# marcin119a/vae-los-angeles

Hardware: AMD Instinct MI355X
Metric: training samples/sec, MultiModalVAE batch 65536 (higher is better)
Workload: dtype bf16

## Files before the change

vae-los-angeles_amd/csrc/gemm_nt2.h:

```cpp
#pragma once
#include "common.h"
#include "gemm_nt_epi.h"

namespace mm {

template <int WN> struct Nt2Lds {
    static constexpr int A_BYTES = TILE * ROW_BYTES;
    static constexpr int W_BYTES = 64 * WN * ROW_BYTES;
    static constexpr int SLOT = A_BYTES + W_BYTES;
    static constexpr int RING = 2 * SLOT;
    static constexpr int RED = RING;
    static constexpr int ECOL = RED + 4 * 64 * WN * 4;
    static constexpr int TOTAL = ECOL + 8 * 64 * WN * 4;
};

STAMP_BUFFER(nt2)

typedef __attribute__((address_space(3))) void lds_void;
typedef __attribute__((address_space(1))) const void gbl_void;

template <typename Epi, int WN>
__device__ __forceinline__ void nt2_loss_epilogue(unsigned char* smem, const float* ecol, float* red, f32x4 (&acc)[4][4], const Epi& epi,
                                                  int row0, int col0, int M, int N, int tid, int lane, int wr, int wc)
{
    static_assert(WN == 2, "128 x 128 tiles: the fp32 tile is exactly the 64 KB ring");
    const int li = lane & 15, lg = lane >> 4;
    const int c = tid & 31, r0 = tid >> 5;
    const int colg = col0 + 4 * c;
    typedef typename Epi::t_t TT;
    const TT* __restrict__ T = epi.T;
    bf16* __restrict__ G = epi.G;
    const bool interior = row0 + TILE <= M && col0 + 128 <= N;
    float t[16][4];
    if (interior) {
#pragma unroll
        for (int i = 0; i < 16; ++i) {
            const TT* tp = T + (long)(row0 + r0 + 8 * i) * epi.ldt + colg;
#pragma unroll
            for (int e = 0; e < 4; e += Epi::VT) VLoad<TT, Epi::VT>::ld(tp + e, &t[i][e]);
        }
    } else {
#pragma unroll
        for (int i = 0; i < 16; ++i) {
            const TT* tp = T + (long)min(row0 + r0 + 8 * i, M - 1) * epi.ldt;
#pragma unroll
            for (int e = 0; e < 4; e += Epi::VT) VLoad<TT, Epi::VT>::ld(tp + min(colg + e, N - Epi::VT), &t[i][e]);
        }
    }
    __syncthreads();
#pragma unroll
    for (int m = 0; m < 4; ++m)
#pragma unroll
        for (int n = 0; n < 4; ++n) {
            const int row = wr * 64 + m * 16 + li, ch = 16 * wc + 4 * n + lg;
            *(f32x4*)(smem + row * 512 + ((ch ^ (row & 7)) << 4)) = acc[m][n];
        }
    __syncthreads();
    const int gcols = (int)min((long)((N + 7) & ~7), epi.ldg);
    const unsigned char* src = smem + r0 * 512 + ((c ^ (r0 & 7)) << 4);
    const f32x2 b01 = {ecol[4 * c], ecol[4 * c + 1]}, b23 = {ecol[4 * c + 2], ecol[4 * c + 3]};
    f32x2 lsum2 = {0.f, 0.f};
    if (interior) {
#pragma unroll
        for (int i = 0; i < 16; ++i) {
            const f32x4 z = *(const f32x4*)(src + i * 8 * 512);
            f32x2 g01, g23;
            lsum2 += epi.term2(f32x2{z[0], z[1]} + b01, f32x2{t[i][0], t[i][1]}, g01);
            lsum2 += epi.term2(f32x2{z[2], z[3]} + b23, f32x2{t[i][2], t[i][3]}, g23);
            const bf16x4 o = {(bf16)g01[0], (bf16)g01[1], (bf16)g23[0], (bf16)g23[1]};
            *(bf16x4*)(G + (long)(row0 + r0 + 8 * i) * epi.ldg + colg) = o;
        }
    } else {
#pragma unroll
        for (int i = 0; i < 16; ++i) {
            const int grow = row0 + r0 + 8 * i;
            const f32x4 z = *(const f32x4*)(src + i * 8 * 512);
            f32x2 g01, g23;
            const f32x2 l01 = epi.term2(f32x2{z[0], z[1]} + b01, f32x2{t[i][0], t[i][1]}, g01);
            const f32x2 l23 = epi.term2(f32x2{z[2], z[3]} + b23, f32x2{t[i][2], t[i][3]}, g23);
            const float l[4] = {l01[0], l01[1], l23[0], l23[1]}, ge[4] = {g01[0], g01[1], g23[0], g23[1]};
            float g[4];
#pragma unroll
            for (int e = 0; e < 4; ++e) {
                const bool ok = grow < M && colg + e < N;
                lsum2[e & 1] += ok ? l[e] : 0.f;
                g[e] = ok ? ge[e] : 0.f;
            }
            if (grow < M && colg < gcols) {
                bf16x4 o;
#pragma unroll
                for (int e = 0; e < 4; ++e) o[e] = (bf16)g[e];
                *(bf16x4*)(G + (long)grow * epi.ldg + colg) = o;
            }
        }
    }
    const float lsum = lsum2[0] + lsum2[1];
    const float ws = wave_sum(lsum);
    if (lane == 0) red[tid >> 6] = ws;
    __syncthreads();
    if (tid == 0) {
        const double v = (double)red[0] + (double)red[1] + (double)red[2] + (double)red[3];
        if (v != 0.0) unsafeAtomicAdd(epi.sum, v);
    }
}

template <typename Epi, int WN>
__device__ __forceinline__ void nt2_relumask_epilogue(unsigned char* smem, f32x4 (&acc)[4][4], const Epi& epi,
                                                      int row0, int col0, int M, int N, int tid, int lane, int wr, int wc)
{
    static_assert(WN == 2, "128 x 128 tiles: the fp32 tile is exactly the 64 KB ring");
    const int li = lane & 15, lg = lane >> 4;
    const int c = tid & 31, r0 = tid >> 5;
    const int colg = col0 + 4 * c;
    const bf16* __restrict__ H = epi.H;
    bf16* __restrict__ C = epi.C;
    const int ch_ = min(colg, ((N + 7) & ~7) - 4);
    bf16x4 hv[16];
#pragma unroll
    for (int i = 0; i < 16; ++i) hv[i] = *(const bf16x4*)(H + (long)min(row0 + r0 + 8 * i, M - 1) * epi.ldh + ch_);
    __syncthreads();
#pragma unroll
    for (int m = 0; m < 4; ++m)
#pragma unroll
        for (int n = 0; n < 4; ++n) {
            const int row = wr * 64 + m * 16 + li, ch = 16 * wc + 4 * n + lg;
            *(f32x4*)(smem + row * 512 + ((ch ^ (row & 7)) << 4)) = acc[m][n];
        }
    __syncthreads();
    const int ccols = (int)min((long)((N + 7) & ~7), epi.ldc);
    const unsigned char* src = smem + r0 * 512 + ((c ^ (r0 & 7)) << 4);
#pragma unroll
    for (int i = 0; i < 16; ++i) {
        const int grow = row0 + r0 + 8 * i;
        const f32x4 z = *(const f32x4*)(src + i * 8 * 512);
        bf16x4 o;
#pragma unroll
        for (int e = 0; e < 4; ++e) o[e] = (bf16)((colg + e < N && (float)hv[i][e] > 0.f) ? z[e] : 0.f);
        if (grow < M && colg < ccols) *(bf16x4*)(C + (long)grow * epi.ldc + colg) = o;
    }
    __syncthreads();
}

template <typename Epi, int WN>
__device__ __forceinline__ void nt2_bnbwd_epilogue(unsigned char* smem, const float* ecol, float* red, f32x4 (&acc)[4][4], const Epi& epi,
                                                   int row0, int col0, int M, int N, int tid, int lane, int wr, int wc)
{
    static_assert(WN == 2, "128 x 128 tiles: the fp32 tile is exactly the 64 KB ring");
    constexpr int BN = 128;
    const int li = lane & 15, lg = lane >> 4;
    const int c = tid & 31, r0 = tid >> 5;
    const int colg = col0 + 4 * c;
    const bf16* __restrict__ Y = epi.Y;
    const uint8_t* __restrict__ K_ = epi.mask;
    bf16* __restrict__ C = epi.C;
    const bool has_mask = K_ != nullptr;
    const int cy = min(colg, ((N + 7) & ~7) - 4);
    bf16x4 yv[16]; uint32_t mv[16];
#pragma unroll
    for (int i = 0; i < 16; ++i) {
        const long grow = min(row0 + r0 + 8 * i, M - 1);
        yv[i] = *(const bf16x4*)(Y + grow * epi.ldy + cy);
        mv[i] = has_mask ? *(const uint32_t*)(K_ + grow * epi.ldm + min(colg, ((N + 3) & ~3) - 4)) : 0x01010101u;
    }
    __syncthreads();
#pragma unroll
    for (int m = 0; m < 4; ++m)
#pragma unroll
        for (int n = 0; n < 4; ++n) {
            const int row = wr * 64 + m * 16 + li, ch = 16 * wc + 4 * n + lg;
            *(f32x4*)(smem + row * 512 + ((ch ^ (row & 7)) << 4)) = acc[m][n];
        }
    __syncthreads();
    const int ccols = (int)min((long)((N + 7) & ~7), epi.ldc);
    const unsigned char* src = smem + r0 * 512 + ((c ^ (r0 & 7)) << 4);
    float sc[4], sh[4], mu[4], rs[4], s1[4] = {0.f, 0.f, 0.f, 0.f}, s2[4] = {0.f, 0.f, 0.f, 0.f};
#pragma unroll
    for (int e = 0; e < 4; ++e) { sc[e] = ecol[4 * c + e]; sh[e] = ecol[BN + 4 * c + e]; mu[e] = ecol[2 * BN + 4 * c + e]; rs[e] = ecol[3 * BN + 4 * c + e]; }
#pragma unroll
    for (int i = 0; i < 16; ++i) {
        const int grow = row0 + r0 + 8 * i;
        const f32x4 z = *(const f32x4*)(src + i * 8 * 512);
        bf16x4 o;
#pragma unroll
        for (int e = 0; e < 4; ++e) {
            const bool ok = grow < M && colg + e < N;
            const float y = (float)yv[i][e];
            const float keep = ((mv[i] >> (8 * e)) & 0xffu) ? epi.inv_keep : 0.f;
            const float d = (ok && y * sc[e] + sh[e] > 0.f) ? z[e] * (has_mask ? keep : 1.f) : 0.f;
            const float xh = (y - mu[e]) * rs[e];
            s1[e] += d; s2[e] += d * xh;
            o[e] = (bf16)d;
        }
        if (grow < M && colg < ccols) *(bf16x4*)(C + (long)grow * epi.ldc + colg) = o;
    }
    __syncthreads();
    float* part = (float*)smem;
#pragma unroll
    for (int e = 0; e < 4; ++e) { part[(r0 * 2 + 0) * BN + 4 * c + e] = s1[e]; part[(r0 * 2 + 1) * BN + 4 * c + e] = s2[e]; }
    __syncthreads();
    if (tid < 2 * BN) {
        const int which = tid >> 7, col = tid & (BN - 1);
        float v = 0.f;
#pragma unroll
        for (int g = 0; g < 8; ++g) v += part[(g * 2 + which) * BN + col];
        if (col0 + col < N) unsafeAtomicAdd((which ? epi.stat2 : epi.stat1) + col0 + col, (double)v);
    }
    __syncthreads();
}

template <typename Epi, int WN>
__global__ __launch_bounds__(128 * WN, 2)
void gemm_nt2_kernel(const bf16* __restrict__ A, long lda, const bf16* __restrict__ W, long ldw, int M, int N, int K, int gx, int gy, Epi epi)
{
    typedef bf16 CT;
    typedef Nt2Lds<WN> LD;
    constexpr int BK = 64, BN = 64 * WN, NW = 2 * WN;
    constexpr int A_PIECES = TILE / 8, W_PIECES = BN / 8;
    constexpr int A_PER = A_PIECES / NW, W_PER = W_PIECES / NW;
    typedef Mma<CT>::frag frag;
    typedef EpiCols<sizeof(typename Epi::out_t) == 2> EC;
    extern __shared__ __attribute__((aligned(16))) unsigned char smem[];
    float* red = (float*)(smem + LD::RED);
    float* ecol = (float*)(smem + LD::ECOL);

    const int tid = threadIdx.x, lane = tid & 63, wid = __builtin_amdgcn_readfirstlane(tid >> 6);
    const int wr = wid / WN, wc = wid % WN;
    const int nk = (K + BK - 1) / BK;
    const int kmax = ((K + 7) & ~7) - 8;
    const int ntiles = ((gx + 7) / 8) * 8 * gy;

    auto tile_rc = [&](int T, int& rt, int& ct) { const int slot = T >> 3; ct = slot % gy; rt = (slot / gy) * 8 + (T & 7); };
    auto next_tile = [&](int T) {
        for (T += gridDim.x; T < ntiles; T += gridDim.x) { int rt, ct; tile_rc(T, rt, ct); if (rt < gx) return T; }
        return -1;
    };
    int T = blockIdx.x;
    { int rt, ct; tile_rc(T, rt, ct); if (rt >= gx) T = next_tile(T); }
    if (T < 0) return;
    const int prow = lane >> 3, ppos = lane & 7;
    auto issue = [&](int tile, int kt, int slot) {
        int rt, ct; tile_rc(tile, rt, ct);
        const int row0 = rt * TILE, col0 = ct * BN;
        unsigned char* sA = smem + slot * LD::SLOT;
        unsigned char* sW = sA + LD::A_BYTES;
        const bf16* Ak = A + kt * BK;
        const bf16* Wk = W + kt * BK;
#pragma unroll
        for (int i = 0; i < A_PER; ++i) {
            const int p = wid + NW * i;
            const int r = p * 8 + prow;
            const int c = ppos ^ (r & 7);
            const int kc = min(c * 8, kmax - kt * BK);
            const unsigned off = (unsigned)min(row0 + r, M - 1) * (unsigned)lda + (unsigned)kc;
            __builtin_amdgcn_global_load_lds((gbl_void*)(Ak + off), (lds_void*)(sA + p * 1024), 16, 0, 0);
        }
#pragma unroll
        for (int i = 0; i < W_PER; ++i) {
            const int p = wid + NW * i, r = p * 8 + prow;
            const int c = ppos ^ (r & 7);
            const int wrw = (r & ~63) + EC::wrow(r & 63);
            const unsigned off = (unsigned)(col0 + wrw) * (unsigned)ldw + (unsigned)(c * 8);
            __builtin_amdgcn_global_load_lds((gbl_void*)(Wk + off), (lds_void*)(sW + p * 1024), 16, 0, 0);
        }
    };

    f32x4 acc[4][4];
    frag f0a[4], f0b[4], f1a[4], f1b[4];
    auto rd = [&](frag (&af)[4], frag (&bf)[4], int slot, int s) {
        const unsigned char* sA = smem + slot * LD::SLOT;
        const unsigned char* sW = sA + LD::A_BYTES;
        const int ch = s * 4 + (lane >> 4);
#pragma unroll
        for (int m = 0; m < 4; ++m) {
            const int r = wr * 64 + m * 16 + (lane & 15);
            af[m] = *(const frag*)(sA + r * ROW_BYTES + ((ch ^ (r & 7)) << 4));
        }
#pragma unroll
        for (int n = 0; n < 4; ++n) { const int r = wc * 64 + n * 16 + (lane & 15); bf[n] = *(const frag*)(sW + r * ROW_BYTES + ((ch ^ (r & 7)) << 4)); }
    };
    auto mma = [&](const frag (&af)[4], const frag (&bf)[4]) {
#pragma unroll
        for (int m = 0; m < 4; ++m)
#pragma unroll
            for (int n = 0; n < 4; ++n) Mma<CT>::mma(acc[m][n], bf[n], af[m]);
    };

    STAMP_ONLY(unsigned long long st_acc[10] = {}; STAMP_T(t_begin);)
    issue(T, 0, 0);
    int g = 0;
    for (;;) {
        const int Tn = next_tile(T);
        int rt, ct; tile_rc(T, rt, ct);
        const int row0 = rt * TILE, col0 = ct * BN;
#pragma unroll
        for (int m = 0; m < 4; ++m)
#pragma unroll
            for (int n = 0; n < 4; ++n) acc[m][n] = f32x4{0.f, 0.f, 0.f, 0.f};
        EpiOperands<Epi> eops;
        for (int kt = 0; kt < nk; ++kt, ++g) {
            STAMP_T(t0);
            asm volatile("s_waitcnt vmcnt(0)" ::: "memory");
            STAMP_T(t1);
            __syncthreads();
            STAMP_T(t2);
            if (kt == 0) nt_epilogue_fill_cols<Epi, WN>(ecol, epi, col0, N, tid);
            if (kt + 1 < nk) issue(T, kt + 1, (g + 1) & 1);
            else if (Tn >= 0 && !Epi::LDS_STREAM) issue(Tn, 0, (g + 1) & 1);
            STAMP_T(t3);
            rd(f0a, f0b, g & 1, 0);
            rd(f1a, f1b, g & 1, 1);
            mma(f0a, f0b);
            mma(f1a, f1b);
            STAMP_ONLY(asm volatile("s_nop 0" :: "v"(acc[0][0][0]), "v"(acc[3][3][3])));
            STAMP_T(t4);
            STAMP_ADD(0, t1 - t0); STAMP_ADD(1, t2 - t1); STAMP_ADD(2, t3 - t2); STAMP_ADD(3, t4 - t3); STAMP_ADD(4, 1);
        }
        STAMP_T(te0);
        if (nk == 1) __syncthreads();
        if constexpr (Epi::LDS_STREAM) {
            if constexpr (Epi::MODE == 2) nt2_bnbwd_epilogue<Epi, WN>(smem, ecol, red, acc, epi, row0, col0, M, N, tid, lane, wr, wc);
            else if constexpr (Epi::MODE == 3) nt2_relumask_epilogue<Epi, WN>(smem, acc, epi, row0, col0, M, N, tid, lane, wr, wc);
            else nt2_loss_epilogue<Epi, WN>(smem, ecol, red, acc, epi, row0, col0, M, N, tid, lane, wr, wc);
            if (Tn >= 0) issue(Tn, 0, g & 1);
        } else {
            nt_epilogue_prefetch<Epi, 0>(eops, epi, row0, col0, M, N, BN, lane, wr, wc);
            nt_epilogue<CT, Epi, WN>(red, ecol, acc, epi, eops, row0, col0, M, N, tid, lane, wr, wc);
        }
        STAMP_T(te1);
        STAMP_ADD(9, te1 - te0);
        if (Tn < 0) break;
        T = Tn;
    }
    STAMP_T(t_end);
    STAMP_ADD(5, 1); STAMP_ADD(6, t_end - t_begin);
    STAMP_ONLY(if (tid == 0 && (blockIdx.x & 15) == 3) stamp_flush(stamps_nt2, st_acc));
}

template <typename Epi, int WN>
static int launch_nt2(const void* A, long lda, const void* W, long ldw, int M, int N, int K, const Epi& epi, hipStream_t st) {
    const int gx = (M + TILE - 1) / TILE, gy = (N + 64 * WN - 1) / (64 * WN);
    const int ntiles = ((gx + 7) / 8) * 8 * gy;
    int grid = NUM_CU * (WN == 2 ? 2 : 1);
    if (grid > ntiles) grid = ntiles;
    return launch_lds<gemm_nt2_kernel<Epi, WN>>(dim3(grid), dim3(128 * WN), Nt2Lds<WN>::TOTAL, st,
                                                (const bf16*)A, lda, (const bf16*)W, ldw, M, N, K, gx, gy, epi);
}

}
```

vae-los-angeles_amd/csrc/gemm_nt_epi.h:

```cpp
#pragma once
#include "common.h"
#include "wave_slab.h"

namespace mm {

template <typename OT, bool STATS_>
struct EpiStore {
    static constexpr bool STATS = STATS_;
    static constexpr bool LDS_STREAM = false;
    static constexpr int NEED = 0;
    typedef OT out_t; typedef OT h_t;
    OT* C; long ldc; const float* bias; int act; int accumulate;
    const OT* H; long ldh; const uint8_t* mask; long ldm;
    double* stat1; double* stat2;
    struct Col { float b; };
    static constexpr int NCOL = 1;
    __device__ __forceinline__ bool stores() const { return true; }
    __device__ __forceinline__ bool accum() const { return accumulate != 0; }
    bool accumulate_requested() const { return accumulate != 0; }
    __device__ __forceinline__ void fill(float* e, int BN, int cl, int c, int N) const { e[cl] = (bias && c < N) ? bias[c] : 0.f; }
    __device__ __forceinline__ Col col(const float* e, int BN, int cl) const { return Col{e[cl]}; }
    __device__ __forceinline__ int act_code() const { return act; }
    template <int ACT>
    __device__ __forceinline__ float compute(float v, float, unsigned, const Col& cc, bool count, float& s1, float& s2) const {
        v += cc.b;
        const int a = ACT < 0 ? act : ACT;
        if (a == 1) v = fmaxf(v, 0.f);
        else if (a == 2) v = __builtin_amdgcn_rcpf(1.f + __expf(-v));
        const float r = to_f32(from_f32<OT>(v));
        if (STATS && count) { s1 += r; s2 += r * r; }
        return r;
    }
};

template <typename OT, bool STATS>
inline EpiStore<OT, STATS> epi_store(const mmvae_gemm_nt_args* a) {
    return {(OT*)a->c, a->ldc, a->bias, a->act, a->accumulate, nullptr, 0, nullptr, 0, STATS ? a->stat1 : nullptr, STATS ? a->stat2 : nullptr};
}

template <typename OT, typename HT>
struct EpiReluMask {
    static constexpr bool STATS = false;
    static constexpr bool LDS_STREAM = false;
    static constexpr int NEED = 1;
    typedef OT out_t; typedef HT h_t;
    OT* C; long ldc; const HT* H; long ldh; const uint8_t* mask; long ldm;
    double* stat1; double* stat2;
    struct Col {};
    static constexpr int NCOL = 0;
    __device__ __forceinline__ bool stores() const { return true; }
    __device__ __forceinline__ bool accum() const { return false; }
    bool accumulate_requested() const { return false; }
    __device__ __forceinline__ void fill(float*, int, int, int, int) const {}
    __device__ __forceinline__ Col col(const float*, int, int) const { return Col{}; }
    __device__ __forceinline__ int act_code() const { return 0; }
    template <int ACT>
    __device__ __forceinline__ float compute(float v, float h, unsigned, const Col&, bool, float&, float&) const {
        return h > 0.f ? v : 0.f;
    }
};

template <typename OT, typename YT>
struct EpiBnBwd {
    static constexpr bool STATS = true;
    static constexpr bool LDS_STREAM = false;
    static constexpr int NEED = 2;
    typedef OT out_t; typedef YT h_t;
    OT* C; long ldc; const YT* H; long ldh; const uint8_t* mask; long ldm;
    const float* scale; const float* shift; const float* mean; const float* rstd; float inv_keep;
    const float* coef; int phase;
    double* stat1; double* stat2;
    struct Col { float sc, sh, mu, rs, c0, c1, c2; };
    __device__ __forceinline__ bool stores() const { return phase != 0; }
    __device__ __forceinline__ bool accum() const { return false; }
    bool accumulate_requested() const { return false; }
    static constexpr int NCOL = 7;
    __device__ __forceinline__ void fill(float* e, int BN, int cl, int c, int N) const {
        const bool ok = c < N, p1 = ok && phase == 1;
        e[cl] = ok ? scale[c] : 0.f; e[BN + cl] = ok ? shift[c] : 0.f; e[2 * BN + cl] = ok ? mean[c] : 0.f; e[3 * BN + cl] = ok ? rstd[c] : 0.f;
        e[4 * BN + cl] = p1 ? coef[c] : 0.f; e[5 * BN + cl] = p1 ? coef[N + c] : 0.f; e[6 * BN + cl] = p1 ? coef[2 * N + c] : 0.f;
    }
    __device__ __forceinline__ Col col(const float* e, int BN, int cl) const {
        return Col{e[cl], e[BN + cl], e[2 * BN + cl], e[3 * BN + cl], e[4 * BN + cl], e[5 * BN + cl], e[6 * BN + cl]};
    }
    __device__ __forceinline__ int act_code() const { return 0; }
    template <int ACT>
    __device__ __forceinline__ float compute(float v, float y, unsigned mb, const Col& cc, bool count, float& s1, float& s2) const {
        const float keep = mask ? (mb ? inv_keep : 0.f) : 1.f;
        const float d = (y * cc.sc + cc.sh > 0.f) ? v * keep : 0.f;
        const float xh = (y - cc.mu) * cc.rs;
        if (phase != 1) { if (count) { s1 += d; s2 += d * xh; } return d; }
        return cc.c0 * (d - cc.c1 - xh * cc.c2);
    }
};

template <int MODE_, int VT_, typename TT = float>
struct EpiLoss {
    static constexpr bool STATS = false;
    static constexpr bool LDS_STREAM = true;
    static constexpr int NEED = 0;
    static constexpr int MODE = MODE_, VT = VT_;
    typedef float out_t; typedef float h_t;
    typedef TT t_t;
    bf16* G; long ldg; const TT* T; long ldt; const float* bias; double* sum;
    struct Col { float b; };
    static constexpr int NCOL = 1;
    bool accumulate_requested() const { return false; }
    __device__ __forceinline__ void fill(float* e, int BN, int cl, int c, int N) const { e[cl] = (bias && c < N) ? bias[c] : 0.f; }
    __device__ __forceinline__ float term(float x, float t, float& g) const {
        if constexpr (MODE == 0) { const float d = x - t; g = 2.f * d; return d * d; }
        else {
            const float pe = __builtin_amdgcn_rcpf(1.f + __expf(-x));
            const float lp = fmaxf(fast_ln(pe), -100.f), l1p = fmaxf(fast_ln(1.f - pe), -100.f);
            const float pq = (1.f - pe) * pe, d = pe - t;
            g = d * fminf(pq * 1e12f, 1.f);
            return -(t * lp + (1.f - t) * l1p);
        }
    }
    __device__ __forceinline__ f32x2 term2(const f32x2 x, const f32x2 t, f32x2& g) const {
        if constexpr (MODE == 0) { const f32x2 d = x - t; g = d * 2.f; return d * d; }
        else {
            const f32x2 nx = x * -1.4426950408889634f;
            const f32x2 s = f32x2{__builtin_amdgcn_exp2f(nx[0]), __builtin_amdgcn_exp2f(nx[1])} + 1.f;
            const f32x2 pe = {__builtin_amdgcn_rcpf(s[0]), __builtin_amdgcn_rcpf(s[1])};
            const f32x2 om = 1.f - pe;
            f32x2 lp = f32x2{__builtin_amdgcn_logf(pe[0]), __builtin_amdgcn_logf(pe[1])} * 0.6931471805599453f;
            f32x2 l1p = f32x2{__builtin_amdgcn_logf(om[0]), __builtin_amdgcn_logf(om[1])} * 0.6931471805599453f;
            lp = f32x2{fmaxf(lp[0], -100.f), fmaxf(lp[1], -100.f)};
            l1p = f32x2{fmaxf(l1p[0], -100.f), fmaxf(l1p[1], -100.f)};
            const f32x2 pq = om * pe, d = pe - t, c = pq * 1e12f;
            g = d * f32x2{fminf(c[0], 1.f), fminf(c[1], 1.f)};
            return -__builtin_elementwise_fma(1.f - t, l1p, t * lp);
        }
    }
};

struct EpiBnBwdStream {
    static constexpr bool STATS = true;
    static constexpr bool LDS_STREAM = true;
    static constexpr int NEED = 0;
    static constexpr int MODE = 2;
    typedef float out_t; typedef float h_t;
    bf16* C; long ldc; const bf16* Y; long ldy; const uint8_t* mask; long ldm;
    const float* scale; const float* shift; const float* mean; const float* rstd; float inv_keep;
    double* stat1; double* stat2;
    struct Col { float b; };
    static constexpr int NCOL = 4;
    bool accumulate_requested() const { return false; }
    __device__ __forceinline__ void fill(float* e, int BN, int cl, int c, int N) const {
        const bool ok = c < N;
        e[cl] = ok ? scale[c] : 0.f; e[BN + cl] = ok ? shift[c] : 0.f; e[2 * BN + cl] = ok ? mean[c] : 0.f; e[3 * BN + cl] = ok ? rstd[c] : 0.f;
    }
};

struct EpiReluMaskStream {
    static constexpr bool STATS = false;
    static constexpr bool LDS_STREAM = true;
    static constexpr int NEED = 0;
    static constexpr int MODE = 3;
    typedef float out_t; typedef float h_t;
    bf16* C; long ldc; const bf16* H; long ldh;
    struct Col { float b; };
    static constexpr int NCOL = 0;
    bool accumulate_requested() const { return false; }
    __device__ __forceinline__ void fill(float*, int, int, int, int) const {}
};

template <typename Epi>
struct EpiOperands {
    typedef typename Epi::h_t HT;
    typedef EpiCols<sizeof(typename Epi::out_t) == 2> EC;
    static constexpr int HD = EC::G * (int)sizeof(HT) / 4;
    static constexpr int MD = EC::G / 4;
    static_assert(Epi::NEED == 0 || HD == 4, "epilogue operand groups are 16-byte vectors (H and output of the same width)");
    uint32_t h[4 * EC::NG][HD];
    uint32_t mk[4 * EC::NG][MD];
};

template <typename Epi> __device__ __forceinline__ bool epi_h_vec(const Epi& epi) {
    return Epi::NEED >= 1 && (epi.ldh * sizeof(typename Epi::h_t)) % 16 == 0 && ((uintptr_t)epi.H & 15) == 0;
}
template <typename Epi> __device__ __forceinline__ bool epi_h_lines(const Epi& epi, int col0, int BN, int ncols) {
    return epi_h_vec(epi) && (epi.ldh * sizeof(typename Epi::h_t)) % 128 == 0 && ((uintptr_t)epi.H & 127) == 0 && col0 + BN <= ncols;
}
template <typename Epi> __device__ __forceinline__ bool epi_m_vec(const Epi& epi) {
    return Epi::NEED >= 2 && epi.mask != nullptr && epi.ldm % 8 == 0 && ((uintptr_t)epi.mask & 7) == 0;
}

template <typename Epi, int HALF>
__device__ __forceinline__ void nt_epilogue_prefetch(EpiOperands<Epi>& ops, const Epi& epi, int row0, int col0, int M, int N, int BN, int lane, int wr, int wc) {
    typedef EpiOperands<Epi> EO;
    typedef typename EO::EC EC;
    const int li = lane & 15, lg = lane >> 4;
    const int ncols = (N + 7) & ~7;
    if constexpr (Epi::NEED >= 1) {
        if (epi_h_lines(epi, col0, BN, ncols)) {
#pragma unroll
            for (int m = 2 * HALF; m < 2 * HALF + 2; ++m)
#pragma unroll
                for (int g = 0; g < EC::NG; ++g) {
                    const int r = row0 + wr * 64 + m * 16 + (g & 1) * 8 + (li & 7);
                    const int c = col0 + wc * 64 + EC::base((g & ~1) + (li >> 3), lg);
                    const uint4 t = *(const uint4*)(epi.H + (long)min(r, M - 1) * epi.ldh + c);
                    ops.h[m * EC::NG + g][0] = t.x; ops.h[m * EC::NG + g][1] = t.y; ops.h[m * EC::NG + g][2] = t.z; ops.h[m * EC::NG + g][3] = t.w;
                }
        } else if (epi_h_vec(epi)) {
#pragma unroll
            for (int m = 2 * HALF; m < 2 * HALF + 2; ++m) {
                const long ro = (long)min(row0 + wr * 64 + m * 16 + li, M - 1) * epi.ldh;
#pragma unroll
                for (int g = 0; g < EC::NG; ++g) {
                    const int c = col0 + wc * 64 + EC::base(g, lg);
                    const uint4 t = *(const uint4*)(epi.H + ro + (c + EC::G <= ncols ? c : 0));
                    ops.h[m * EC::NG + g][0] = t.x; ops.h[m * EC::NG + g][1] = t.y; ops.h[m * EC::NG + g][2] = t.z; ops.h[m * EC::NG + g][3] = t.w;
                }
            }
        }
    }
    if constexpr (Epi::NEED >= 2) {
        if (epi_m_vec(epi)) {
#pragma unroll
            for (int m = 2 * HALF; m < 2 * HALF + 2; ++m) {
                const long ro = (long)min(row0 + wr * 64 + m * 16 + li, M - 1) * epi.ldm;
#pragma unroll
                for (int g = 0; g < EC::NG; ++g) {
                    const int c = col0 + wc * 64 + EC::base(g, lg);
                    const uint8_t* q = epi.mask + ro + (c + EC::G <= ncols ? c : 0);
                    if constexpr (EO::MD == 2) { const uint2 t = *(const uint2*)q; ops.mk[m * EC::NG + g][0] = t.x; ops.mk[m * EC::NG + g][1] = t.y; }
                    else ops.mk[m * EC::NG + g][0] = *(const uint32_t*)q;
                }
            }
        }
    }
}

template <typename Epi, int WN>
__device__ __forceinline__ void nt_epilogue_fill_cols(float* ecol, const Epi& epi, int col0, int N, int tid) {
    constexpr int BN = 64 * WN;
    if (Epi::NCOL > 0 && tid < BN) epi.fill(ecol, BN, tid, col0 + tid, N);
}

template <typename Epi, int ACT, bool ACCUM, bool VEC>
__device__ __forceinline__ void nt_epilogue_body(const float* ecol, f32x4 (&acc)[4][4], const Epi& epi, const EpiOperands<Epi>& ops,
                                                 float* red, bool want_stats, int BN, int row0, int col0, int M, int N, int lane, int wr, int wc,
                                                 int tile_rows = TILE)
{
    typedef typename Epi::out_t OT;
    typedef typename Epi::h_t HT;
    typedef EpiOperands<Epi> EO;
    typedef typename EO::EC EC;
    constexpr int G = EC::G, NG = EC::NG;
    constexpr int EPCO = 16 / (int)sizeof(OT);
    const int li = lane & 15, lg = lane >> 4;
    const int n_store = (int)min((long)((N + EPCO - 1) / EPCO * EPCO), epi.ldc);
    const bool c16 = (epi.ldc * sizeof(OT)) % 16 == 0 && ((uintptr_t)epi.C & 15) == 0;
    const bool c8 = (epi.ldc * sizeof(OT)) % 8 == 0 && ((uintptr_t)epi.C & 7) == 0;
    const bool has_mask = Epi::NEED >= 2 && epi.mask != nullptr;
    const bool full_lines = !ACCUM && epi.stores() && row0 + tile_rows <= M && col0 + BN <= n_store &&
                            (epi.ldc * sizeof(OT)) % 128 == 0 && ((uintptr_t)epi.C & 127) == 0;
    const unsigned low = (li & 8) ? 0u : 0xffffffffu;
    const bool h_lines = VEC && Epi::NEED >= 1 && epi_h_lines(epi, col0, BN, (N + 7) & ~7);
#pragma unroll
    for (int p = 0; p < NG / 2; ++p) {
        float s1[2][G], s2[2][G];
#pragma unroll
        for (int h = 0; h < 2; ++h)
#pragma unroll
            for (int e = 0; e < G; ++e) { s1[h][e] = 0.f; s2[h][e] = 0.f; }
#pragma unroll
        for (int m = 0; m < 4; ++m) {
            const int row = row0 + wr * 64 + m * 16 + li;
            const bool rok = row < M;
            uint32_t pk[2][4];
            uint32_t hw[2][4];
            if constexpr (Epi::NEED >= 1 && VEC) {
#pragma unroll
                for (int q = 0; q < 4; ++q) {
                    const uint32_t l0 = ops.h[m * NG + 2 * p][q], l1 = ops.h[m * NG + 2 * p + 1][q];
                    hw[0][q] = l0; hw[1][q] = l1;
                    if (h_lines) {
                        const uint32_t got = (uint32_t)__builtin_amdgcn_mov_dpp((int)((l1 & low) | (l0 & ~low)), 0x128, 0xf, 0xf, true);
                        hw[0][q] = (l0 & low) | (got & ~low);
                        hw[1][q] = (got & low) | (l1 & ~low);
                    }
                }
            }
#pragma unroll
            for (int h = 0; h < 2; ++h) {
                const int g = 2 * p + h;
                const int cw = wc * 64 + EC::base(g, lg), c0 = col0 + cw;
                float hv[G]; unsigned mb[G]; float o[G];
#pragma unroll
                for (int e = 0; e < G; ++e) { hv[e] = 0.f; mb[e] = 1u; o[e] = 0.f; }
                if constexpr (Epi::NEED >= 1) {
                    if constexpr (VEC) {
#pragma unroll
                        for (int e = 0; e < G; ++e) {
                            if constexpr (sizeof(HT) == 2) {
                                const uint32_t w = hw[h][e >> 1];
                                hv[e] = __uint_as_float((e & 1) ? (w & 0xffff0000u) : (w << 16));
                            } else hv[e] = __uint_as_float(hw[h][e]);
                        }
                    } else {
#pragma unroll
                        for (int e = 0; e < G; ++e) if (rok && c0 + e < N) hv[e] = to_f32(epi.H[(long)row * epi.ldh + c0 + e]);
                    }
                }
                if constexpr (Epi::NEED >= 2) {
                    if constexpr (VEC) {
                        if (has_mask) {
#pragma unroll
                            for (int e = 0; e < G; ++e) mb[e] = (ops.mk[m * NG + g][e >> 2] >> (8 * (e & 3))) & 0xffu;
                        }
                    } else if (has_mask) {
#pragma unroll
                        for (int e = 0; e < G; ++e) if (rok && c0 + e < N) mb[e] = epi.mask[(long)row * epi.ldm + c0 + e];
                    }
                }
                OT* gp = epi.C + (long)row * epi.ldc + c0;
                if constexpr (ACCUM) {
#pragma unroll
                    for (int e = 0; e < G; ++e) if (rok && c0 + e < N) o[e] = to_f32(gp[e]);
                }
#pragma unroll
                for (int e = 0; e < G; ++e) {
                    const int n = EC::tile(g, e), j = e & 3;
                    const bool ok = rok && (c0 + e < N);
                    const typename Epi::Col cc = epi.col(ecol, BN, cw + e);
                    float v = epi.template compute<ACT>(acc[m][n][j], hv[e], mb[e], cc, ok, s1[h][e], s2[h][e]);
                    if constexpr (ACCUM) v += o[e];
                    o[e] = (c0 + e < N) ? v : 0.f;
                }
                if constexpr (sizeof(OT) == 2) {
#pragma unroll
                    for (int q = 0; q < 4; ++q) {
                        const uint32_t lo = __float_as_uint(to_f32(from_f32<OT>(o[2 * q]))), hi = __float_as_uint(to_f32(from_f32<OT>(o[2 * q + 1])));
                        pk[h][q] = (lo >> 16) | (hi & 0xffff0000u);
                    }
                } else {
#pragma unroll
                    for (int q = 0; q < 4; ++q) pk[h][q] = __float_as_uint(o[q]);
                }
                if (!full_lines && epi.stores() && rok && c0 < n_store) {
                    const bool whole = c0 + G <= n_store;
                    if (whole && c16) *(uint4*)gp = uint4{pk[h][0], pk[h][1], pk[h][2], pk[h][3]};
                    else if (sizeof(OT) == 4 && whole && c8) { ((uint2*)gp)[0] = uint2{pk[h][0], pk[h][1]}; ((uint2*)gp)[1] = uint2{pk[h][2], pk[h][3]}; }
                    else {
#pragma unroll
                        for (int e = 0; e < G; ++e) if (c0 + e < n_store) gp[e] = from_f32<OT>(o[e]);
                    }
                }
            }
            if (full_lines) {
                uint32_t st0[4], st1[4];
#pragma unroll
                for (int q = 0; q < 4; ++q) {
                    const uint32_t send = (pk[1][q] & low) | (pk[0][q] & ~low);
                    const uint32_t got = (uint32_t)__builtin_amdgcn_mov_dpp((int)send, 0x128, 0xf, 0xf, true);
                    st0[q] = (pk[0][q] & low) | (got & ~low);
                    st1[q] = (got & low) | (pk[1][q] & ~low);
                }
                const int rbase = row0 + wr * 64 + m * 16 + (li & 7);
                const int cd = col0 + wc * 64 + EC::base(2 * p + (li >> 3), lg);
                *(uint4*)(epi.C + (long)rbase * epi.ldc + cd) = uint4{st0[0], st0[1], st0[2], st0[3]};
                *(uint4*)(epi.C + (long)(rbase + 8) * epi.ldc + cd) = uint4{st1[0], st1[1], st1[2], st1[3]};
            }
        }
        if (Epi::STATS && want_stats) {
#pragma unroll
            for (int h = 0; h < 2; ++h) {
                const int cw = wc * 64 + EC::base(2 * p + h, lg);
                float v[2 * G];
#pragma unroll
                for (int e = 0; e < G; ++e) { v[e] = s1[h][e]; v[G + e] = s2[h][e]; }
                int bit = 8;
#pragma unroll
                for (int half = G; half >= 1; half >>= 1, bit >>= 1) {
                    const unsigned up = (li & bit) ? 0xffffffffu : 0u;
#pragma unroll
                    for (int i = 0; i < half; ++i) {
                        const unsigned lo = __float_as_uint(v[i]), hi = __float_as_uint(v[i + half]);
                        const float keep = __uint_as_float((hi & up) | (lo & ~up));
                        const float send = __uint_as_float((lo & up) | (hi & ~up));
                        v[i] = keep + __shfl_xor(send, bit, 64);
                    }
                }
                if constexpr (G == 4) v[0] += __shfl_xor(v[0], 1, 64);
                const int which = li >> 3;
                const int e = G == 8 ? (li & 7) : ((li >> 1) & 3);
                if (G == 8 || (li & 1) == 0) red[(wr * 2 + which) * BN + cw + e] = v[0];
            }
        }
    }
}

template <typename CT, typename Epi, int WN = 2>
__device__ __forceinline__ void nt_epilogue(float* red, const float* ecol, f32x4 (&acc)[4][4], const Epi& epi, EpiOperands<Epi>& ops,
                                            int row0, int col0, int M, int N, int tid, int lane, int wr, int wc)
{
    constexpr int BN = 64 * WN;
    typedef EpiOperands<Epi> EO;
    typedef typename EO::EC EC;
    const bool want_stats = Epi::STATS && (epi.stat1 != nullptr || epi.stat2 != nullptr);
    const bool vec = (Epi::NEED < 1 || epi_h_vec(epi)) && (Epi::NEED < 2 || epi.mask == nullptr || epi_m_vec(epi));
    if (epi.accum()) {
        nt_epilogue_body<Epi, -1, true, false>(ecol, acc, epi, ops, red, want_stats, BN, row0, col0, M, N, lane, wr, wc);
    } else if (!vec) {
        nt_epilogue_body<Epi, -1, false, false>(ecol, acc, epi, ops, red, want_stats, BN, row0, col0, M, N, lane, wr, wc);
    } else {
        nt_epilogue_prefetch<Epi, 1>(ops, epi, row0, col0, M, N, BN, lane, wr, wc);
        const int a = epi.act_code();
        if (a == 0) nt_epilogue_body<Epi, 0, false, true>(ecol, acc, epi, ops, red, want_stats, BN, row0, col0, M, N, lane, wr, wc);
        else if (a == 1) nt_epilogue_body<Epi, 1, false, true>(ecol, acc, epi, ops, red, want_stats, BN, row0, col0, M, N, lane, wr, wc);
        else nt_epilogue_body<Epi, 2, false, true>(ecol, acc, epi, ops, red, want_stats, BN, row0, col0, M, N, lane, wr, wc);
    }
    if (want_stats) {
        __syncthreads();
        if (tid < BN && col0 + tid < N) {
            if (epi.stat1) unsafeAtomicAdd(epi.stat1 + col0 + tid, (double)(red[0 * BN + tid] + red[2 * BN + tid]));
            if (epi.stat2) unsafeAtomicAdd(epi.stat2 + col0 + tid, (double)(red[1 * BN + tid] + red[3 * BN + tid]));
        }
    }
}

}
```

Before: 54.16 million.

## Stream GEMM epilogue through half-tile LDS slot to overlap next tile's operand loads

```diff
diff --git a/vae-los-angeles_amd/csrc/gemm_nt2.h b/vae-los-angeles_amd/csrc/gemm_nt2.h
--- a/vae-los-angeles_amd/csrc/gemm_nt2.h
+++ b/vae-los-angeles_amd/csrc/gemm_nt2.h
@@ -19,8 +19,104 @@
 typedef __attribute__((address_space(3))) void lds_void;
 typedef __attribute__((address_space(1))) const void gbl_void;
 
-template <typename Epi, int WN>
-__device__ __forceinline__ void nt2_loss_epilogue(unsigned char* smem, const float* ecol, float* red, f32x4 (&acc)[4][4], const Epi& epi,
+__device__ __forceinline__ void nt2_lds_barrier() {
+    asm volatile("s_waitcnt lgkmcnt(0)" ::: "memory");
+    __builtin_amdgcn_s_barrier();
+    asm volatile("" ::: "memory");
+}
+
+__device__ __forceinline__ void nt2_operands_landed() { __builtin_amdgcn_s_waitcnt(0x0F70); }
+
+__device__ __forceinline__ void nt2_stream_put(unsigned char* slot, const f32x4 (&acc)[4][4], int h, int lane, int wr, int wc)
+{
+    const int li = lane & 15, lg = lane >> 4;
+    nt2_lds_barrier();
+    if (wr == h) {
+#pragma unroll
+        for (int m = 0; m < 4; ++m)
+#pragma unroll
+            for (int n = 0; n < 4; ++n) {
+                const int row = m * 16 + li, ch = 16 * wc + 4 * n + lg;
+                *(f32x4*)(slot + row * 512 + ((ch ^ (row & 7)) << 4)) = acc[m][n];
+            }
+    }
+    nt2_lds_barrier();
+}
+
+template <bool INTERIOR, typename Epi>
+__device__ __forceinline__ f32x2 nt2_loss_rows(unsigned char* slot, const float* ecol, f32x4 (&acc)[4][4], const Epi& epi,
+                                               int row0, int col0, int M, int N, int tid, int lane, int wr, int wc)
+{
+    const int c = tid & 31, r0 = tid >> 5;
+    const int colg = col0 + 4 * c;
+    typedef typename Epi::t_t TT;
+    const TT* __restrict__ T = epi.T;
+    bf16* __restrict__ G = epi.G;
+    float t[16][4];
+#pragma unroll
+    for (int i = 0; i < 16; ++i) {
+        const TT* tp = T + (long)(INTERIOR ? row0 + r0 + 8 * i : min(row0 + r0 + 8 * i, M - 1)) * epi.ldt;
+#pragma unroll
+        for (int e = 0; e < 4; e += Epi::VT) VLoad<TT, Epi::VT>::ld(tp + (INTERIOR ? colg + e : min(colg + e, N - Epi::VT)), &t[i][e]);
+    }
+    const int gcols = (int)min((long)((N + 7) & ~7), epi.ldg);
+    const unsigned char* src = slot + r0 * 512 + ((c ^ (r0 & 7)) << 4);
+    f32x2 lsum2 = {0.f, 0.f}, b01, b23;
+#pragma unroll
+    for (int i = 0; i < 16; ++i) {
+        if ((i & 7) == 0) nt2_stream_put(slot, acc, i >> 3, lane, wr, wc);
+        if (i == 0) { nt2_operands_landed(); b01 = f32x2{ecol[4 * c], ecol[4 * c + 1]}; b23 = f32x2{ecol[4 * c + 2], ecol[4 * c + 3]}; }
+        const int grow = row0 + r0 + 8 * i;
+        const f32x4 z = *(const f32x4*)(src + (i & 7) * 8 * 512);
+        f32x2 g01, g23;
+        const f32x2 l01 = epi.term2(f32x2{z[0], z[1]} + b01, f32x2{t[i][0], t[i][1]}, g01);
+        const f32x2 l23 = epi.term2(f32x2{z[2], z[3]} + b23, f32x2{t[i][2], t[i][3]}, g23);
+        if constexpr (INTERIOR) {
+            lsum2 += l01;
+            lsum2 += l23;
+            const bf16x4 o = {(bf16)g01[0], (bf16)g01[1], (bf16)g23[0], (bf16)g23[1]};
+            *(bf16x4*)(G + (long)grow * epi.ldg + colg) = o;
+        } else {
+            const float l[4] = {l01[0], l01[1], l23[0], l23[1]}, ge[4] = {g01[0], g01[1], g23[0], g23[1]};
+            float g[4];
+#pragma unroll
+            for (int e = 0; e < 4; ++e) {
+                const bool ok = grow < M && colg + e < N;
+                lsum2[e & 1] += ok ? l[e] : 0.f;
+                g[e] = ok ? ge[e] : 0.f;
+            }
+            if (grow < M && colg < gcols) {
+                bf16x4 o;
+#pragma unroll
+                for (int e = 0; e < 4; ++e) o[e] = (bf16)g[e];
+                *(bf16x4*)(G + (long)grow * epi.ldg + colg) = o;
+            }
+        }
+    }
+    return lsum2;
+}
+
+template <typename Epi, int WN>
+__device__ __forceinline__ void nt2_loss_epilogue(unsigned char* slot, const float* ecol, float* red, f32x4 (&acc)[4][4], const Epi& epi,
+                                                  int row0, int col0, int M, int N, int tid, int lane, int wr, int wc)
+{
+    static_assert(WN == 2, "128 x 128 tiles: half of the fp32 tile is exactly one 32 KB ring slot");
+    const bool interior = row0 + TILE <= M && col0 + 128 <= N;
+    f32x2 lsum2;
+    if (interior) lsum2 = nt2_loss_rows<true>(slot, ecol, acc, epi, row0, col0, M, N, tid, lane, wr, wc);
+    else lsum2 = nt2_loss_rows<false>(slot, ecol, acc, epi, row0, col0, M, N, tid, lane, wr, wc);
+    const float lsum = lsum2[0] + lsum2[1];
+    const float ws = wave_sum(lsum);
+    if (lane == 0) red[tid >> 6] = ws;
+    nt2_lds_barrier();
+    if (tid == 0) {
+        const double v = (double)red[0] + (double)red[1] + (double)red[2] + (double)red[3];
+        if (v != 0.0) unsafeAtomicAdd(epi.sum, v);
+    }
+}
+
+template <typename Epi, int WN>
+__device__ __forceinline__ void nt2_loss_epilogue_whole(unsigned char* smem, const float* ecol, float* red, f32x4 (&acc)[4][4], const Epi& epi,
                                                   int row0, int col0, int M, int N, int tid, int lane, int wr, int wc)
 {
     static_assert(WN == 2, "128 x 128 tiles: the fp32 tile is exactly the 64 KB ring");
@@ -47,7 +143,7 @@
             for (int e = 0; e < 4; e += Epi::VT) VLoad<TT, Epi::VT>::ld(tp + min(colg + e, N - Epi::VT), &t[i][e]);
         }
     }
-    __syncthreads();
+    nt2_lds_barrier();
 #pragma unroll
     for (int m = 0; m < 4; ++m)
 #pragma unroll
@@ -55,7 +151,7 @@
             const int row = wr * 64 + m * 16 + li, ch = 16 * wc + 4 * n + lg;
             *(f32x4*)(smem + row * 512 + ((ch ^ (row & 7)) << 4)) = acc[m][n];
         }
-    __syncthreads();
+    nt2_lds_barrier();
     const int gcols = (int)min((long)((N + 7) & ~7), epi.ldg);
     const unsigned char* src = smem + r0 * 512 + ((c ^ (r0 & 7)) << 4);
     const f32x2 b01 = {ecol[4 * c], ecol[4 * c + 1]}, b23 = {ecol[4 * c + 2], ecol[4 * c + 3]};
@@ -97,7 +193,7 @@
     const float lsum = lsum2[0] + lsum2[1];
     const float ws = wave_sum(lsum);
     if (lane == 0) red[tid >> 6] = ws;
-    __syncthreads();
+    nt2_lds_barrier();
     if (tid == 0) {
         const double v = (double)red[0] + (double)red[1] + (double)red[2] + (double)red[3];
         if (v != 0.0) unsafeAtomicAdd(epi.sum, v);
@@ -105,11 +201,10 @@
 }
 
 template <typename Epi, int WN>
-__device__ __forceinline__ void nt2_relumask_epilogue(unsigned char* smem, f32x4 (&acc)[4][4], const Epi& epi,
+__device__ __forceinline__ void nt2_relumask_epilogue(unsigned char* slot, f32x4 (&acc)[4][4], const Epi& epi,
                                                       int row0, int col0, int M, int N, int tid, int lane, int wr, int wc)
 {
-    static_assert(WN == 2, "128 x 128 tiles: the fp32 tile is exactly the 64 KB ring");
-    const int li = lane & 15, lg = lane >> 4;
+    static_assert(WN == 2, "128 x 128 tiles: half of the fp32 tile is exactly one 32 KB ring slot");
     const int c = tid & 31, r0 = tid >> 5;
     const int colg = col0 + 4 * c;
     const bf16* __restrict__ H = epi.H;
@@ -118,36 +213,27 @@
     bf16x4 hv[16];
 #pragma unroll
     for (int i = 0; i < 16; ++i) hv[i] = *(const bf16x4*)(H + (long)min(row0 + r0 + 8 * i, M - 1) * epi.ldh + ch_);
-    __syncthreads();
-#pragma unroll
-    for (int m = 0; m < 4; ++m)
-#pragma unroll
-        for (int n = 0; n < 4; ++n) {
-            const int row = wr * 64 + m * 16 + li, ch = 16 * wc + 4 * n + lg;
-            *(f32x4*)(smem + row * 512 + ((ch ^ (row & 7)) << 4)) = acc[m][n];
-        }
-    __syncthreads();
     const int ccols = (int)min((long)((N + 7) & ~7), epi.ldc);
-    const unsigned char* src = smem + r0 * 512 + ((c ^ (r0 & 7)) << 4);
+    const unsigned char* src = slot + r0 * 512 + ((c ^ (r0 & 7)) << 4);
 #pragma unroll
     for (int i = 0; i < 16; ++i) {
+        if ((i & 7) == 0) nt2_stream_put(slot, acc, i >> 3, lane, wr, wc);
+        if (i == 0) nt2_operands_landed();
         const int grow = row0 + r0 + 8 * i;
-        const f32x4 z = *(const f32x4*)(src + i * 8 * 512);
+        const f32x4 z = *(const f32x4*)(src + (i & 7) * 8 * 512);
         bf16x4 o;
 #pragma unroll
         for (int e = 0; e < 4; ++e) o[e] = (bf16)((colg + e < N && (float)hv[i][e] > 0.f) ? z[e] : 0.f);
         if (grow < M && colg < ccols) *(bf16x4*)(C + (long)grow * epi.ldc + colg) = o;
     }
-    __syncthreads();
-}
-
-template <typename Epi, int WN>
-__device__ __forceinline__ void nt2_bnbwd_epilogue(unsigned char* smem, const float* ecol, float* red, f32x4 (&acc)[4][4], const Epi& epi,
+}
+
+template <typename Epi, int WN>
+__device__ __forceinline__ void nt2_bnbwd_epilogue(unsigned char* slot, const float* ecol, float* red, f32x4 (&acc)[4][4], const Epi& epi,
                                                    int row0, int col0, int M, int N, int tid, int lane, int wr, int wc)
 {
-    static_assert(WN == 2, "128 x 128 tiles: the fp32 tile is exactly the 64 KB ring");
+    static_assert(WN == 2, "128 x 128 tiles: half of the fp32 tile is exactly one 32 KB ring slot");
     constexpr int BN = 128;
-    const int li = lane & 15, lg = lane >> 4;
     const int c = tid & 31, r0 = tid >> 5;
     const int colg = col0 + 4 * c;
     const bf16* __restrict__ Y = epi.Y;
@@ -162,24 +248,19 @@
         yv[i] = *(const bf16x4*)(Y + grow * epi.ldy + cy);
         mv[i] = has_mask ? *(const uint32_t*)(K_ + grow * epi.ldm + min(colg, ((N + 3) & ~3) - 4)) : 0x01010101u;
     }
-    __syncthreads();
-#pragma unroll
-    for (int m = 0; m < 4; ++m)
-#pragma unroll
-        for (int n = 0; n < 4; ++n) {
-            const int row = wr * 64 + m * 16 + li, ch = 16 * wc + 4 * n + lg;
-            *(f32x4*)(smem + row * 512 + ((ch ^ (row & 7)) << 4)) = acc[m][n];
-        }
-    __syncthreads();
     const int ccols = (int)min((long)((N + 7) & ~7), epi.ldc);
-    const unsigned char* src = smem + r0 * 512 + ((c ^ (r0 & 7)) << 4);
+    const unsigned char* src = slot + r0 * 512 + ((c ^ (r0 & 7)) << 4);
     float sc[4], sh[4], mu[4], rs[4], s1[4] = {0.f, 0.f, 0.f, 0.f}, s2[4] = {0.f, 0.f, 0.f, 0.f};
 #pragma unroll
-    for (int e = 0; e < 4; ++e) { sc[e] = ecol[4 * c + e]; sh[e] = ecol[BN + 4 * c + e]; mu[e] = ecol[2 * BN + 4 * c + e]; rs[e] = ecol[3 * BN + 4 * c + e]; }
-#pragma unroll
     for (int i = 0; i < 16; ++i) {
+        if ((i & 7) == 0) nt2_stream_put(slot, acc, i >> 3, lane, wr, wc);
+        if (i == 0) {
+            nt2_operands_landed();
+#pragma unroll
+            for (int e = 0; e < 4; ++e) { sc[e] = ecol[4 * c + e]; sh[e] = ecol[BN + 4 * c + e]; mu[e] = ecol[2 * BN + 4 * c + e]; rs[e] = ecol[3 * BN + 4 * c + e]; }
+        }
         const int grow = row0 + r0 + 8 * i;
-        const f32x4 z = *(const f32x4*)(src + i * 8 * 512);
+        const f32x4 z = *(const f32x4*)(src + (i & 7) * 8 * 512);
         bf16x4 o;
 #pragma unroll
         for (int e = 0; e < 4; ++e) {
@@ -193,11 +274,11 @@
         }
         if (grow < M && colg < ccols) *(bf16x4*)(C + (long)grow * epi.ldc + colg) = o;
     }
-    __syncthreads();
-    float* part = (float*)smem;
+    nt2_lds_barrier();
+    float* part = (float*)slot;
 #pragma unroll
     for (int e = 0; e < 4; ++e) { part[(r0 * 2 + 0) * BN + 4 * c + e] = s1[e]; part[(r0 * 2 + 1) * BN + 4 * c + e] = s2[e]; }
-    __syncthreads();
+    nt2_lds_barrier();
     if (tid < 2 * BN) {
         const int which = tid >> 7, col = tid & (BN - 1);
         float v = 0.f;
@@ -205,8 +286,9 @@
         for (int g = 0; g < 8; ++g) v += part[(g * 2 + which) * BN + col];
         if (col0 + col < N) unsafeAtomicAdd((which ? epi.stat2 : epi.stat1) + col0 + col, (double)v);
     }
-    __syncthreads();
-}
+}
+
+template <typename Epi> constexpr bool nt2_stream_halves() { if constexpr (Epi::LDS_STREAM) return Epi::STREAM_HALVES; else return false; }
 
 template <typename Epi, int WN>
 __global__ __launch_bounds__(128 * WN, 2)
@@ -288,6 +370,8 @@
     STAMP_ONLY(unsigned long long st_acc[10] = {}; STAMP_T(t_begin);)
     issue(T, 0, 0);
     int g = 0;
+    constexpr bool HALVES = nt2_stream_halves<Epi>();
+    bool landed = false;
     for (;;) {
         const int Tn = next_tile(T);
         int rt, ct; tile_rc(T, rt, ct);
@@ -299,9 +383,9 @@
         EpiOperands<Epi> eops;
         for (int kt = 0; kt < nk; ++kt, ++g) {
             STAMP_T(t0);
-            asm volatile("s_waitcnt vmcnt(0)" ::: "memory");
+            if (!(HALVES && kt == 0 && landed)) asm volatile("s_waitcnt vmcnt(0)" ::: "memory");
             STAMP_T(t1);
-            __syncthreads();
+            if constexpr (HALVES) nt2_lds_barrier(); else __syncthreads();
             STAMP_T(t2);
             if (kt == 0) nt_epilogue_fill_cols<Epi, WN>(ecol, epi, col0, N, tid);
             if (kt + 1 < nk) issue(T, kt + 1, (g + 1) & 1);
@@ -314,14 +398,19 @@
             STAMP_ONLY(asm volatile("s_nop 0" :: "v"(acc[0][0][0]), "v"(acc[3][3][3])));
             STAMP_T(t4);
             STAMP_ADD(0, t1 - t0); STAMP_ADD(1, t2 - t1); STAMP_ADD(2, t3 - t2); STAMP_ADD(3, t4 - t3); STAMP_ADD(4, 1);
+            STAMP_ADD(7, kt == 0 ? t1 - t0 : 0); STAMP_ADD(8, kt == 0 ? 1 : 0);
         }
         STAMP_T(te0);
-        if (nk == 1) __syncthreads();
+        if (nk == 1 && !Epi::LDS_STREAM) __syncthreads();
         if constexpr (Epi::LDS_STREAM) {
-            if constexpr (Epi::MODE == 2) nt2_bnbwd_epilogue<Epi, WN>(smem, ecol, red, acc, epi, row0, col0, M, N, tid, lane, wr, wc);
-            else if constexpr (Epi::MODE == 3) nt2_relumask_epilogue<Epi, WN>(smem, acc, epi, row0, col0, M, N, tid, lane, wr, wc);
-            else nt2_loss_epilogue<Epi, WN>(smem, ecol, red, acc, epi, row0, col0, M, N, tid, lane, wr, wc);
-            if (Tn >= 0) issue(Tn, 0, g & 1);
+            if (Tn >= 0 && HALVES) issue(Tn, 0, g & 1);
+            unsigned char* slot = HALVES ? smem + ((g - 1) & 1) * LD::SLOT : smem;
+            if constexpr (Epi::MODE == 2) nt2_bnbwd_epilogue<Epi, WN>(slot, ecol, red, acc, epi, row0, col0, M, N, tid, lane, wr, wc);
+            else if constexpr (Epi::MODE == 3) nt2_relumask_epilogue<Epi, WN>(slot, acc, epi, row0, col0, M, N, tid, lane, wr, wc);
+            else if constexpr (!HALVES) nt2_loss_epilogue_whole<Epi, WN>(slot, ecol, red, acc, epi, row0, col0, M, N, tid, lane, wr, wc);
+            else nt2_loss_epilogue<Epi, WN>(slot, ecol, red, acc, epi, row0, col0, M, N, tid, lane, wr, wc);
+            landed = true;
+            if (Tn >= 0 && !HALVES) issue(Tn, 0, g & 1);
         } else {
             nt_epilogue_prefetch<Epi, 0>(eops, epi, row0, col0, M, N, BN, lane, wr, wc);
             nt_epilogue<CT, Epi, WN>(red, ecol, acc, epi, eops, row0, col0, M, N, tid, lane, wr, wc);
diff --git a/vae-los-angeles_amd/csrc/gemm_nt_epi.h b/vae-los-angeles_amd/csrc/gemm_nt_epi.h
--- a/vae-los-angeles_amd/csrc/gemm_nt_epi.h
+++ b/vae-los-angeles_amd/csrc/gemm_nt_epi.h
@@ -98,6 +98,7 @@
 struct EpiLoss {
     static constexpr bool STATS = false;
     static constexpr bool LDS_STREAM = true;
+    static constexpr bool STREAM_HALVES = MODE_ != 1;
     static constexpr int NEED = 0;
     static constexpr int MODE = MODE_, VT = VT_;
     typedef float out_t; typedef float h_t;
@@ -138,6 +139,7 @@
 struct EpiBnBwdStream {
     static constexpr bool STATS = true;
     static constexpr bool LDS_STREAM = true;
+    static constexpr bool STREAM_HALVES = true;
     static constexpr int NEED = 0;
     static constexpr int MODE = 2;
     typedef float out_t; typedef float h_t;
@@ -156,6 +158,7 @@
 struct EpiReluMaskStream {
     static constexpr bool STATS = false;
     static constexpr bool LDS_STREAM = true;
+    static constexpr bool STREAM_HALVES = true;
     static constexpr int NEED = 0;
     static constexpr int MODE = 3;
     typedef float out_t; typedef float h_t;
```

After: 54.43 million (median of 6 runs). Within noise of the previous version (+0.5%).
